# doesburg11/PredPreyGrass

Hardware: NVIDIA B200
Metric: agent_steps_per_s_incl_obs (higher is better)
Workload: dtype f64

## Files before the change

### predpreygrass_b200/csrc/ppg_api.cu

```cuda
#include <cuda_runtime.h>

#include <algorithm>
#include <cmath>
#include <cstdio>
#include <cstdlib>
#include <cstring>
#include <string>
#include <vector>

#include "ppg_device.cuh"

namespace ppg {
cudaError_t launch_step_base(const StepParams& p, int warps_per_cta, int n_cta, size_t smem, cudaStream_t stream);
cudaError_t step_base_occupancy(int warps_per_cta, int map_bytes, bool bulk, bool split, size_t smem, int* blocks_per_sm);
cudaError_t launch_prepare_offsets(const EnvHdr* hdr, int B, int n0, int n1, unsigned long long* cntA, unsigned long long* sum1,
                                   unsigned long long* sum2, int32_t* totals4, unsigned epoch, int hdr_founders, cudaStream_t s);
cudaError_t launch_init_hdr(EnvHdr* hdr, int B, unsigned long long seed, cudaStream_t s);
cudaError_t launch_relabel_rows(const StepParams& p, const unsigned long long* cntA, const unsigned long long* sum1,
                                const unsigned long long* sum2, const int32_t* totals4, cudaStream_t s);
cudaError_t launch_mark_reset(EnvHdr* hdr, int B, const unsigned long long* seeds, const uint8_t* mask, cudaStream_t s);
cudaError_t launch_set_tape(EnvHdr* hdr, int B, const long long* cell_off, cudaStream_t s);
cudaError_t launch_random_actions(const int32_t* n_rows, const int32_t* re0, const int32_t* ra0, const int32_t* re1,
                                  const int32_t* ra1, int32_t* a0, int32_t* a1, unsigned long long seed, unsigned call,
                                  unsigned n_actions, unsigned env_base, int blocks, cudaStream_t s);
// ... 6 lines not shown
cudaError_t launch_eco_founders(const StepParams& p, cudaStream_t s);
cudaError_t launch_step_stag(const StepParams& p, int n_cta, size_t smem, cudaStream_t stream);
cudaError_t step_stag_occupancy(int map_bytes, bool split, size_t smem, int* blocks_per_sm);
cudaError_t launch_set_tape_reals_stag(StagHdr* shdr, int B, const long long* real_off, cudaStream_t s);
cudaError_t launch_random_actions_stag(const int32_t* n_rows, const int32_t* re0, const int32_t* ra0, const int32_t* re1, const int32_t* ra1,
                                       int32_t* a0, int32_t* a1, unsigned long long seed, unsigned call, unsigned env_base, int t2_pred,
                                       int t2_prey, int ar0, int ar1, int blocks, cudaStream_t s);
}

namespace ppg { int g_pdl_chain = -1; }

using namespace ppg;

__global__ void ppg_pow_selftest_kernel(const double* __restrict__ x, const double* __restrict__ y, double* __restrict__ out, long long n) {
  for (long long i = (long long)blockIdx.x * blockDim.x + threadIdx.x; i < n; i += (long long)gridDim.x * blockDim.x) out[i] = ppg_pow(x[i], y[i]);
}

struct ppg_handle_s {
  ppg_config cfg;
  int B = 0, device = 0;
  StepParams P;
  std::vector<int32_t> walls;
  int warps_per_cta = 4, n_cta = 0;
  size_t smem_bytes = 0;
  unsigned long long launches_step = 0;
  unsigned long long ticket_next = 0;
  unsigned long long obs_ticket_next = 0;
  int n_cta_obs = 0;
  bool obs_overlap = true;
  unsigned long long q_next = 0;
  bool profiling = false;
  std::vector<cudaEvent_t> prof_events;
  unsigned long long calls = 0;
  int64_t launch_count = 0;
  std::vector<void*> allocs;
  unsigned long long* d_stats = nullptr;
  int32_t* d_tape_cells = nullptr;
  long long* d_tape_off = nullptr;
  double* d_tape_reals = nullptr;
  long long* d_tape_real_off = nullptr;
  uint8_t* d_mask = nullptr;
  unsigned long long* d_seeds = nullptr;
  int32_t* d_act[2] = {nullptr, nullptr};
  int32_t h_n_rows[4] = {0, 0, 0, 0};
  bool h_n_rows_valid = false;
  ppg_buffers bufs;
  size_t state_bytes = 0;
  std::string err;
};

static thread_local std::string g_err;

#define CK(call)                                                                             \
  do {                                                                                       \
    cudaError_t _e = (call);                                                                 \
    if (_e != cudaSuccess) {                                                                 \
      h->err = std::string(#call) + ": " + cudaGetErrorString(_e);                           \
      return PPG_ERR_CUDA;                                                                   \
    }                                                                                        \
  } while (0)

template <typename T>
static cudaError_t dalloc(ppg_handle h, T** p, size_t n) {
  void* q = nullptr;
  cudaError_t e = cudaMalloc(&q, std::max<size_t>(n, 1) * sizeof(T));
  if (e != cudaSuccess) return e;
// ... 409 lines not shown
    if (lpt) { for (int q = 0; q < 2; ++q) CKC(dalloc(h, &P.perm[q], (size_t)B)); CKC(dalloc(h, &P.perm_tag, 2)); CKC(dalloc(h, &P.perm_cursor, 4)); CKC(cudaMemset(P.perm_tag, 0xFF, 2 * sizeof(unsigned))); }
  }
  if (eco) {
    CKC(dalloc(h, &P.ehdr, (size_t)B));
    if (c.track_episode_sums) CKC(dalloc(h, &P.ep_sums, (size_t)B * PPG_EP_STRIDE));
    CKC(dalloc(h, &P.gh_n, (size_t)B)); CKC(dalloc(h, &P.gh_cell, (size_t)B * PPG_MAX_GHOSTS)); CKC(dalloc(h, &P.gh_val, (size_t)B * PPG_MAX_GHOSTS));
  }
  if (stag) CKC(dalloc(h, &P.shdr, (size_t)B));
  CKC(dalloc(h, &P.gr_pos, (size_t)B * std::max(1, P.n_grass)));
  CKC(dalloc(h, &P.gr_e, (size_t)B * std::max(1, P.n_grass)));
  CKC(dalloc(h, &P.counters, (size_t)B * PPG_N_STATS));
  CKC(dalloc(h, &P.ticket, 1));
  CKC(dalloc(h, &P.env_cycles, (size_t)B));
  if (P.obs_split) {
    void* q = nullptr;
    CKC(cudaMalloc(&q, (size_t)B * (size_t)P.img_stride));
    h->allocs.push_back(q);
    P.obs_img = static_cast<unsigned char*>(q);
    for (int s = 0; s < 2; ++s) CKC(dalloc(h, &P.nb_info[s], (size_t)B * P.cap[s]));
    CKC(dalloc(h, &P.obs_ticket, 1));
    CKC(dalloc(h, &P.queue, (size_t)B));
    CKC(dalloc(h, &P.q_tail, 1));
    if (const char* ev = getenv("PPG_OBS_OVERLAP")) h->obs_overlap = atoi(ev) != 0;
    if (eco)
      for (int s = 0; s < 2; ++s) CKC(dalloc(h, &P.born_obs[s], (size_t)B * PPG_BORN_K * (size_t)P.elems[s]));
    int per_sm = 0, n_sm = 0;
    CKC(obs_occupancy(P, &per_sm));
    CKC(cudaDeviceGetAttribute(&n_sm, cudaDevAttrMultiProcessorCount, device));
    if (per_sm < 1) { h->err = "observation kernel does not fit on an SM"; return fail(PPG_ERR_INVALID); }
    h->n_cta_obs = std::min(B, per_sm * n_sm);
    if (const char* ev = getenv("PPG_OBS_CTAS_PER_SM")) h->n_cta_obs = std::max(1, std::min(h->n_cta_obs, atoi(ev) * n_sm));
    if (const char* ev = getenv("PPG_STEP_CTAS_PER_SM")) h->n_cta = std::max(1, std::min(h->n_cta, atoi(ev) * n_sm));
  }
  CKC(dalloc(h, &P.error, 1));
  CKC(dalloc(h, &h->d_stats, PPG_N_STATS));
  CKC(dalloc(h, &h->d_mask, (size_t)B));
  CKC(dalloc(h, &h->d_seeds, (size_t)B));
  ppg_buffers& b = h->bufs;
  memset(&b, 0, sizeof b);
  for (int s = 0; s < 2; ++s) {
    const size_t rows = (size_t)B * P.cap[s];
    b.row_capacity[s] = (int64_t)rows;
    b.obs_row_elems[s] = P.elems[s];
    void* q = nullptr;
    CKC(cudaMalloc(&q, rows * (size_t)P.elems[s] * sizeof(float)));
    h->allocs.push_back(q);
    P.obs[s] = b.obs[s] = static_cast<float*>(q);
    CKC(dalloc(h, &P.row_env[s], rows)); CKC(dalloc(h, &P.row_agent[s], rows));
    CKC(dalloc(h, &P.reward[s], rows)); CKC(dalloc(h, &P.flags[s], rows));
    CKC(dalloc(h, &P.old_off[s], (size_t)B + 1)); CKC(dalloc(h, &P.new_off[s], (size_t)B + 1));
    CKC(dalloc(h, &P.new_cnt[s], (size_t)B + 1));
    CKC(dalloc(h, &h->d_act[s], rows));
    b.row_env[s] = P.row_env[s]; b.row_agent[s] = P.row_agent[s]; b.reward[s] = P.reward[s]; b.flags[s] = P.flags[s];
    b.old_off[s] = P.old_off[s]; b.new_off[s] = P.new_off[s]; b.new_cnt[s] = P.new_cnt[s];
  }
  CKC(dalloc(h, &P.n_rows, 4)); CKC(dalloc(h, &P.env_flags, (size_t)B)); CKC(dalloc(h, &P.env_status, (size_t)B));
  CKC(dalloc(h, &P.env_step, (size_t)B)); CKC(dalloc(h, &P.env_count, (size_t)B * 2));
  b.n_rows = P.n_rows; b.env_flags = P.env_flags; b.env_status = P.env_status; b.env_step = P.env_step; b.env_count = P.env_count;
  b.n_envs = B;
  CKC(launch_init_hdr(P.hdr, B, c.seed, 0));
  h->launch_count++;
  CKC(cudaDeviceSynchronize());
  *out = h;
  return PPG_OK;
#undef CKC
}
// ... 27 lines not shown
    h->P.tape_cells = h->d_tape_cells;
  }
  CK(launch_set_tape(h->P.hdr, h->B, h->d_tape_off, 0));
  h->launch_count++;
  if (h->P.variant == PPG_VARIANT_ECO || h->P.variant == PPG_VARIANT_STAG) {
    if (h->d_tape_reals) { cudaFree(h->d_tape_reals); h->d_tape_reals = nullptr; }
    if (h->d_tape_real_off) { cudaFree(h->d_tape_real_off); h->d_tape_real_off = nullptr; }
    h->P.tape_reals = nullptr;
    if (t && t->reals && t->real_off) {
      const int64_t total = t->real_off[h->B];
      CK(cudaMalloc(&h->d_tape_reals, sizeof(double) * (size_t)std::max<int64_t>(total, 1)));
      CK(cudaMalloc(&h->d_tape_real_off, sizeof(long long) * ((size_t)h->B + 1)));
      CK(cudaMemcpy(h->d_tape_reals, t->reals, sizeof(double) * (size_t)total, cudaMemcpyHostToDevice));
      CK(cudaMemcpy(h->d_tape_real_off, t->real_off, sizeof(long long) * ((size_t)h->B + 1), cudaMemcpyHostToDevice));
      h->P.tape_reals = h->d_tape_reals;
    }
    if (h->P.variant == PPG_VARIANT_ECO) CK(launch_set_tape_reals(h->P.ehdr, h->B, h->d_tape_real_off, 0));
    else CK(launch_set_tape_reals_stag(h->P.shdr, h->B, h->d_tape_real_off, 0));
    h->launch_count++;
  }
  CK(cudaDeviceSynchronize());
  return PPG_OK;
}

static int prepare_offsets(ppg_handle h, cudaStream_t st) {
  const unsigned prev_epoch = (unsigned)h->launches_step;
  const int q = (int)(prev_epoch & 1u);
  CK(launch_prepare_offsets(h->P.hdr, h->B, h->P.n_init[0], h->P.n_init[1], h->P.cntA[q], h->P.sum1[q], h->P.sum2[q],
                            h->P.totals + 4 * q, prev_epoch, h->P.variant == PPG_VARIANT_ECO && ppg_random_founders(h->P.trait_mode), st));
  h->launch_count++;
  return PPG_OK;
}

static int run_step_kernel(ppg_handle h, const int32_t* a0, const int32_t* a1, const int32_t* o0, const int32_t* o1, cudaStream_t st) {
  StepParams& P = h->P;
  P.actions[0] = a0; P.actions[1] = a1;
  P.order[0] = o0; P.order[1] = o1;
  P.ticket_base = h->ticket_next;
  P.static_first = (h->warps_per_cta == 1 && P.obs_split && P.variant != PPG_VARIANT_ECO) ? 1 : 0;
  if (const char* ev = getenv("PPG_STATIC_FIRST")) P.static_first = P.static_first && atoi(ev) != 0;
  h->ticket_next += P.static_first ? (unsigned long long)h->B
                    : h->warps_per_cta == 1 ? (unsigned long long)h->B + (unsigned long long)h->n_cta
                                          : (unsigned long long)((h->B + h->warps_per_cta - 1) / h->warps_per_cta) + (unsigned long long)h->n_cta;
  P.epoch = (unsigned)(h->launches_step + 1);
  P.q_base = h->q_next;
  if (P.obs_split) h->q_next += (unsigned long long)h->B;
  cudaEvent_t pe[3] = {nullptr, nullptr, nullptr};
  if (h->profiling) {
    for (int k = 0; k < 3; ++k) { CK(cudaEventCreate(&pe[k])); h->prof_events.push_back(pe[k]); }
    CK(cudaEventRecord(pe[0], st));
  }
  if (P.variant == PPG_VARIANT_ECO) CK(launch_step_eco(P, h->n_cta, h->smem_bytes, st));
  else if (P.variant == PPG_VARIANT_STAG) CK(launch_step_stag(P, h->n_cta, h->smem_bytes, st));
  else CK(launch_step_base(P, h->warps_per_cta, h->n_cta, h->smem_bytes, st));
  h->launches_step++;
  h->launch_count++;
  if (h->profiling) CK(cudaEventRecord(pe[1], st));
  if (P.obs_split) {
    P.obs_ticket_base = h->obs_ticket_next;
    h->obs_ticket_next += (unsigned long long)h->B + (unsigned long long)h->n_cta_obs;
    CK(launch_obs(P, h->n_cta_obs, h->obs_overlap && !h->profiling, st));
    h->launch_count++;
  }
  if (h->profiling) CK(cudaEventRecord(pe[2], st));
  h->calls++;
  h->h_n_rows_valid = false;
  return PPG_OK;
}

// ... 86 lines not shown

int ppg_random_actions(ppg_handle h, uint64_t seed, int32_t* actions_pred, int32_t* actions_prey, void* cuda_stream) {
  if (!h || !actions_pred || !actions_prey) return PPG_ERR_INVALID;
  CK(cudaSetDevice(h->device));
  const StepParams& P = h->P;
  if (P.variant == PPG_VARIANT_STAG)
    CK(launch_random_actions_stag(P.n_rows, P.row_env[0], P.row_agent[0], P.row_env[1], P.row_agent[1], actions_pred, actions_prey, seed,
                                  (unsigned)h->calls, (unsigned)P.env_base, P.n_possible_t[0][0], P.n_possible_t[1][0], P.type_ar[0], P.type_ar[1],
                                  148 * 4, static_cast<cudaStream_t>(cuda_stream)));
  else
  CK(launch_random_actions(P.n_rows, P.row_env[0], P.row_agent[0], P.row_env[1], P.row_agent[1], actions_pred, actions_prey,
                           seed, (unsigned)h->calls, (unsigned)P.n_actions, (unsigned)P.env_base, 148 * 4, static_cast<cudaStream_t>(cuda_stream)));
  h->launch_count++;
  return PPG_OK;
}

int ppg_set_pdl_chain(int32_t on) {
  const int before = pdl_chain_enabled() ? 1 : 0;
  g_pdl_chain = on ? 1 : 0;
  return before;
}

int ppg_rollout_random(ppg_handle* handles, int32_t n_handles, void** cuda_streams, int32_t n_steps, uint64_t seed) {
  if (!handles || n_handles <= 0 || n_steps < 0) return PPG_ERR_INVALID;
  struct ChainOff { int before; bool off; ChainOff(bool o) : before(pdl_chain_enabled()), off(o) { if (off) g_pdl_chain = 0; } ~ChainOff() { if (off) g_pdl_chain = before; } } chain_off(n_handles > 1);
  for (int g = 0; g < n_handles; ++g) {
    if (!handles[g]) return PPG_ERR_INVALID;
    if (handles[g]->launches_step == 0) { handles[g]->err = "ppg_rollout_random before ppg_reset"; return PPG_ERR_STATE; }
  }
  for (int k = 0; k < n_steps; ++k)
    for (int g = 0; g < n_handles; ++g) {
      ppg_handle h = handles[g];
      void* st = cuda_streams ? cuda_streams[g] : nullptr;
      int rc = ppg_random_actions(h, seed, h->d_act[0], h->d_act[1], st);
      if (rc) return rc;
      rc = run_step_kernel(h, h->d_act[0], h->d_act[1], nullptr, nullptr, static_cast<cudaStream_t>(st));
      if (rc) return rc;
    }
  return PPG_OK;
}

int ppg_selftest_pow(const double* x, const double* y, double* out, int64_t n, int32_t device) {
  if (!x || !y || !out || n <= 0) return PPG_ERR_INVALID;
  if (cudaSetDevice(device) != cudaSuccess) { g_err = "ppg_selftest_pow: bad device"; return PPG_ERR_NO_DEVICE; }
  double *dx = nullptr, *dy = nullptr, *dz = nullptr;
  const size_t bytes = (size_t)n * sizeof(double);
  cudaError_t e = cudaMalloc(&dx, bytes);
  if (e == cudaSuccess) e = cudaMalloc(&dy, bytes);
  if (e == cudaSuccess) e = cudaMalloc(&dz, bytes);
  if (e == cudaSuccess) e = cudaMemcpy(dx, x, bytes, cudaMemcpyHostToDevice);
  if (e == cudaSuccess) e = cudaMemcpy(dy, y, bytes, cudaMemcpyHostToDevice);
  if (e == cudaSuccess) { ppg_pow_selftest_kernel<<<148 * 8, 256>>>(dx, dy, dz, (long long)n); e = cudaGetLastError(); }
  if (e == cudaSuccess) e = cudaMemcpy(out, dz, bytes, cudaMemcpyDeviceToHost);
  cudaFree(dx); cudaFree(dy); cudaFree(dz);
  if (e != cudaSuccess) { g_err = std::string("ppg_selftest_pow: ") + cudaGetErrorString(e); return PPG_ERR_CUDA; }
  return PPG_OK;
}

int ppg_get_buffers(ppg_handle h, ppg_buffers* out) {
  if (!h || !out) return PPG_ERR_INVALID;
  *out = h->bufs;
  return PPG_OK;
}

struct Seg { void* p; size_t bytes; };
static std::vector<Seg> state_segments(ppg_handle h) {
// ... 323 lines not shown
```

### predpreygrass_b200/csrc/ppg_base.cu

```cuda
#include <cuda_runtime.h>

#include "ppg_step_common.cuh"

#ifndef PPG_MIN_CTAS
#define PPG_MIN_CTAS 20
#endif

namespace ppg {

PHASE_DEFINE(base)
SPAN_DEFINE(base)

#define SEL(a) (s == 0 ? a[0] : a[1])

template <int W, typename MapT, bool BULK, bool SPLIT>
__global__ void __launch_bounds__(W * 32, PPG_MIN_CTAS / W) ppg_step_base_kernel(const __grid_constant__ StepParams p) {
  extern __shared__ __align__(128) unsigned char smem_raw[];
  __shared__ int s_env0;
  const int warp = threadIdx.x >> 5, lane = threadIdx.x & 31;
  SPAN_MARK(base, 0)
  wait_for_stream_predecessor();
  if (SPLIT) allow_dependent_launch();
  unsigned char* const sbase = smem_raw + (size_t)warp * p.smem_per_env;
  const EnvSmem<MapT> S = carve<MapT>(sbase, p);
  const RowDesc D = carve_desc(sbase, p);
  const unsigned sb32 = (unsigned)__cvta_generic_to_shared(sbase);
  const int G = p.G, GG = p.GG, PP = p.P, PS = p.PS;
  const unsigned epoch = p.epoch;
  const int par = (int)(epoch & 1u);
  const int mode_r = p.reward_mode;
  const bool dense = mode_r == PPG_REWARD_DENSE || mode_r == PPG_REWARD_DENSE_ADDITIVE;
  const bool kick = mode_r == PPG_REWARD_SPARSE_KICKBACK;
  const unsigned lt_mask = (1u << lane) - 1u;

  {
    const int n16 = p.init_bytes / 16;
    #pragma unroll 1
    for (int i0 = 0; i0 < n16; i0 += 32 * 8) {
      uint4 v[8];
#pragma unroll
      for (int q = 0; q < 8; ++q) { const int i = i0 + 32 * q + lane; if (i < n16) v[q] = __ldg(reinterpret_cast<const uint4*>(p.init_image) + i); }
#pragma unroll
      for (int q = 0; q < 8; ++q) { const int i = i0 + 32 * q + lane; if (i < n16) reinterpret_cast<uint4*>(sbase + p.so_map[0])[i] = v[q]; }
    }
  }
  unsigned rowctr = 0;
  const int n_old_total[2] = {p.totals[(par ^ 1) * 4 + 0], p.totals[(par ^ 1) * 4 + 1]};
  const int n_blk = (p.B + 31) >> 5, n_grp = (p.B + 1023) >> 10;
// ... 108 lines not shown
            S.pos[s][i] = (uint16_t)((cx << 8) | cy);
            S.E[s][i] = p.init_e[s];
            S.flg[s][i] = F_ALIVE;
            if (kick) S.par[s][i] = 0xFFFF;
            S.ord[s][i] = (uint16_t)i;
            S.map[s][CELLXY(cx, cy)] = (MapT)(i + 1);
          }
          k0 += p.n_init[s];
          n[s] = p.n_init[s];
          h.n_list[s] = (unsigned short)p.n_init[s];
          h.n_sorted[s] = (unsigned short)p.n_init[s];
          h.next_idx[s] = (unsigned short)p.n_init[s];
        }
        #pragma unroll 1
        for (int g = lane; g < p.n_grass; g += 32) {
          const int c = cells[k0 + g];
          const int cx = c / G, cy = c % G;
          S.gpos[g] = (uint16_t)((cx << 8) | cy);
          S.gE[g] = p.grass_cap;
          S.map[2][CELLXY(cx, cy)] = (MapT)(g + 1);
        }
      }
      __syncwarp();
      cur[0] = n[0]; cur[1] = n[1];
      next_live[0] = n[0]; next_live[1] = n[1];
      env_flags = PPG_ENV_RESET;
      PHASE_MARK(2)
    } else if (mode == 2) {
      n[0] = h.n_list[0]; n[1] = h.n_list[1];
      int act_r[3] = {4, 4, 4};
#pragma unroll
      for (int q = 0; q < 3; ++q) {
        const int s = q ? 1 : 0, i = lane + (q == 2 ? 32 : 0);
        if (i < SEL(n)) act_r[q] = p.actions[s][prow_r[q]];
      }
      {
        const double grass_gain = p.season_len > 0 ? p.grass_gain_season[(h.step / p.season_len) & 1] : p.grass_gain;
#pragma unroll
        for (int q = 0; q < 4; ++q) {
          const int g = lane + 32 * q;
          if (g < p.n_grass) {
            S.gpos[g] = (uint16_t)gp_r[q];
            const double v = ge_r[q] + grass_gain;
            S.gE[g] = v < p.grass_cap ? v : p.grass_cap;
            S.map[2][CELLP(gp_r[q])] = (MapT)(g + 1);
          }
        }
        #pragma unroll 1
        for (int g = lane + 128; g < p.n_grass; g += 32) {
          const size_t b = (size_t)env * p.n_grass;
          const unsigned gp = p.gr_pos[b + g];
          S.gpos[g] = (uint16_t)gp;
          const double v = p.gr_e[b + g] + grass_gain;
          S.gE[g] = v < p.grass_cap ? v : p.grass_cap;
          S.map[2][CELLP(gp)] = (MapT)(g + 1);
        }
      }
      PHASE_MARK(4)
      unsigned bad = 0;
      bool resort[2] = {false, false};
#pragma unroll 1
      for (int s = 0; s < 2; ++s) {
        const size_t b = (size_t)env * p.cap[s];
        const int32_t* ordp = p.order[s];
        bool use_order = ordp != nullptr;
        if (PPG_UNLIKELY(use_order)) {
          bool ok = true;
          #pragma unroll 1
          for (int i = lane; i < SEL(n); i += 32) {
            const int d = ordp[p.ag_prow[s][b + i]];
            if ((unsigned)d < (unsigned)SEL(n)) SEL(S.rnk)[d] = (uint16_t)i; else ok = false;
          }
          __syncwarp();
          #pragma unroll 1
          for (int i = lane; i < SEL(n); i += 32) {
            const int d = ordp[p.ag_prow[s][b + i]];
            if ((unsigned)d < (unsigned)SEL(n)) ok &= SEL(S.rnk)[d] == (uint16_t)i;
          }
          use_order = __all_sync(FULL, ok);
          if (!use_order) bad = PPG_STATUS_BAD_ACTION;
          __syncwarp();
        }
        if (s == 0) resort[0] = use_order; else resort[1] = use_order;
        #pragma unroll 1
        for (int i = lane; i < SEL(n); i += 32) {
          const int q = s == 0 ? (i < 32 ? 0 : 3) : (i < 32 ? 1 : (i < 64 ? 2 : 3));
          int prow, a;
          double e;
          unsigned idpos, par16 = 0;
          if (q < 3) {
            prow = q == 0 ? prow_r[0] : (q == 1 ? prow_r[1] : prow_r[2]);
            e = q == 0 ? e_r[0] : (q == 1 ? e_r[1] : e_r[2]);
            idpos = q == 0 ? idpos_r[0] : (q == 1 ? idpos_r[1] : idpos_r[2]);
            a = q == 0 ? act_r[0] : (q == 1 ? act_r[1] : act_r[2]);
            if (kick) par16 = q == 0 ? par_r[0] : (q == 1 ? par_r[1] : par_r[2]);
          } else {
            prow = p.ag_prow[s][b + i];
            e = p.ag_e[s][b + i];
            idpos = (unsigned)p.ag_id[s][b + i] | ((unsigned)p.ag_pos[s][b + i] << 16);
            a = p.actions[s][prow];
            if (kick) par16 = p.ag_par[s][b + i];
          }
          const int d = use_order ? ordp[prow] : i;
          if ((unsigned)a > 8u) { a = 4; bad = PPG_STATUS_BAD_ACTION; }
          SEL(S.id)[d] = (uint16_t)idpos;
          SEL(S.pos)[d] = (uint16_t)(idpos >> 16);
          if (dense) SEL(S.E0)[d] = e;
          SEL(S.E)[d] = e - p.loss[s];
          SEL(S.act)[d] = (uint8_t)a;
          SEL(S.flg)[d] = F_ALIVE;
          SEL(S.ord)[d] = (uint16_t)d;
          SEL(S.rnk)[d] = (uint16_t)d;
          if (kick) { SEL(S.par)[d] = (uint16_t)par16; SEL(S.aux)[d] = 0; }
        }
      }
      h.status |= (unsigned char)__reduce_or_sync(FULL, bad);
      PHASE_MARK(3)
      __syncwarp();
#pragma unroll 1
      for (int s = 0; s < 2; ++s)
        for (int b0 = 0; b0 < SEL(n); b0 += 32) {
          const int i = b0 + lane;
          const bool v = i < SEL(n);
          int cell = 0;
          if (v) { cell = CELLP((unsigned)SEL(S.pos)[i]); SEL(S.map)[cell] = (MapT)(i + 1); }
          __syncwarp();
          bool need = v && SEL(S.map)[cell] < (unsigned)(i + 1);
          while (__any_sync(FULL, need)) {
            if (need) SEL(S.map)[cell] = (MapT)(i + 1);
            __syncwarp();
            need = v && SEL(S.map)[cell] < (unsigned)(i + 1);
          }
        }
// ... 600 lines not shown
  if (e >= B) return;
  EnvHdr h = {};
  h.seed_key = seed;
  h.state = ST_IDLE;
  hdr[e] = h;
}

__global__ void ppg_mark_reset_kernel(EnvHdr* hdr, int B, const unsigned long long* seeds, const uint8_t* mask) {
  const int e = blockIdx.x * blockDim.x + threadIdx.x;
  if (e >= B) return;
  if (mask && !mask[e]) return;
  if (seeds) hdr[e].seed_key = seeds[e];
  hdr[e].state = ST_NEEDS_RESET;
}

__global__ void ppg_set_tape_kernel(EnvHdr* hdr, int B, const long long* cell_off) {
  const int e = blockIdx.x * blockDim.x + threadIdx.x;
  if (e >= B) return;
  hdr[e].tape_pos = cell_off ? cell_off[e] : 0;
  hdr[e].tape_end = cell_off ? cell_off[e + 1] : 0;
}

__global__ void ppg_random_actions_kernel(const int32_t* __restrict__ n_rows, const int32_t* __restrict__ row_env0,
                                          const int32_t* __restrict__ row_agent0, const int32_t* __restrict__ row_env1,
                                          const int32_t* __restrict__ row_agent1, int32_t* act0, int32_t* act1,
                                          unsigned long long seed, unsigned call, unsigned n_actions, unsigned env_base) {
  allow_dependent_launch();
  wait_for_stream_predecessor();
  const volatile int32_t* const nr = n_rows;
  const int n0 = nr[0] + nr[2], n1 = nr[1] + nr[3];
  for (int i = blockIdx.x * blockDim.x + threadIdx.x; i < n0 + n1; i += gridDim.x * blockDim.x) {
    const int s = i >= n0;
    const int row = s ? i - n0 : i;
    const unsigned env = (unsigned)(s ? row_env1[row] : row_env0[row]) + env_base;
    const unsigned id = (unsigned)(s ? row_agent1[row] : row_agent0[row]);
    const unsigned r = ppg_draw_u32(seed, env, call, PPG_STREAM_ACTION + 8u * (unsigned)s, id);
    (s ? act1 : act0)[row] = (int32_t)ppg_bounded(r, n_actions);
  }
}

__global__ void ppg_stats_kernel(const uint32_t* __restrict__ counters, const EnvHdr* __restrict__ hdr, int B,
                                 unsigned long long* out) {
  __shared__ unsigned long long s_acc[PPG_N_STATS];
  if (threadIdx.x < PPG_N_STATS) s_acc[threadIdx.x] = 0;
  __syncthreads();
  const int k = threadIdx.x & (PPG_N_STATS - 1);
  unsigned long long a = 0;
  for (size_t i = (size_t)blockIdx.x * blockDim.x + threadIdx.x; i < (size_t)B * PPG_N_STATS; i += (size_t)gridDim.x * blockDim.x) {
    unsigned v = counters[i];
    if (k == PPG_STAT_STATUS_ENVS) v = hdr[i / PPG_N_STATS].status != 0;
    a += v;
  }
  atomicAdd(&s_acc[k], a);
  __syncthreads();
  if (threadIdx.x < PPG_N_STATS && s_acc[threadIdx.x]) atomicAdd(out + threadIdx.x, s_acc[threadIdx.x]);
}

template <int W, typename MapT, bool BULK, bool SPLIT>
static cudaError_t launch_w(const StepParams& p, int n_cta, size_t smem, cudaStream_t stream) {
  static size_t attr_bytes = 0;
  if (smem > attr_bytes) {
    cudaError_t e = cudaFuncSetAttribute(ppg_step_base_kernel<W, MapT, BULK, SPLIT>, cudaFuncAttributeMaxDynamicSharedMemorySize, (int)smem);
    if (e != cudaSuccess) return e;
    attr_bytes = smem;
  }
  return pdl_launch(ppg_step_base_kernel<W, MapT, BULK, SPLIT>, dim3((unsigned)n_cta), dim3(W * 32), smem, stream, p);
}

template <int W, typename MapT, bool BULK, bool SPLIT>
static cudaError_t occupancy_w(size_t smem, int* blocks_per_sm) {
  cudaError_t e = cudaFuncSetAttribute(ppg_step_base_kernel<W, MapT, BULK, SPLIT>, cudaFuncAttributeMaxDynamicSharedMemorySize, (int)smem);
  if (e != cudaSuccess) return e;
  return cudaOccupancyMaxActiveBlocksPerMultiprocessor(blocks_per_sm, ppg_step_base_kernel<W, MapT, BULK, SPLIT>, W * 32, smem);
}

#define PPG_DISPATCH(FN, ...)                                                                     \
  do {                                                                                            \
    const bool m8 = map_bytes == 1;                                                               \
    if (split) return m8 ? FN<1, uint8_t, false, true>(__VA_ARGS__) : FN<1, uint16_t, false, true>(__VA_ARGS__); \
    if (warps_per_cta == 1) {                                                                     \
      if (bulk) return m8 ? FN<1, uint8_t, true, false>(__VA_ARGS__) : FN<1, uint16_t, true, false>(__VA_ARGS__); \
      return m8 ? FN<1, uint8_t, false, false>(__VA_ARGS__) : FN<1, uint16_t, false, false>(__VA_ARGS__);       \
    }                                                                                             \
    if (warps_per_cta == 4) {                                                                     \
      if (bulk) return m8 ? FN<4, uint8_t, true, false>(__VA_ARGS__) : FN<4, uint16_t, true, false>(__VA_ARGS__); \
      return m8 ? FN<4, uint8_t, false, false>(__VA_ARGS__) : FN<4, uint16_t, false, false>(__VA_ARGS__);       \
    }                                                                                             \
    if (warps_per_cta == 8) {                                                                     \
      if (bulk) return m8 ? FN<8, uint8_t, true, false>(__VA_ARGS__) : FN<8, uint16_t, true, false>(__VA_ARGS__); \
      return m8 ? FN<8, uint8_t, false, false>(__VA_ARGS__) : FN<8, uint16_t, false, false>(__VA_ARGS__);       \
    }                                                                                             \
    return cudaErrorInvalidValue;                                                                 \
  } while (0)

cudaError_t launch_step_base(const StepParams& p, int warps_per_cta, int n_cta, size_t smem, cudaStream_t stream) {
  const int map_bytes = p.map_bytes;
  const bool bulk = p.obs_bulk != 0, split = p.obs_split != 0;
  PPG_DISPATCH(launch_w, p, n_cta, smem, stream);
}

cudaError_t step_base_occupancy(int warps_per_cta, int map_bytes, bool bulk, bool split, size_t smem, int* blocks_per_sm) {
  PPG_DISPATCH(occupancy_w, smem, blocks_per_sm);
}

cudaError_t launch_prepare_offsets(const EnvHdr* hdr, int B, int n0, int n1, unsigned long long* cntA, unsigned long long* sum1,
                                   unsigned long long* sum2, int32_t* totals4, unsigned epoch, int hdr_founders, cudaStream_t s) {
// ... 32 lines not shown
```

### predpreygrass_b200/csrc/ppg_device.cuh

```cuda
#pragma once
#include <cuda_runtime.h>
#include <stdint.h>

#include <cstdlib>
#include <utility>

#include "../../include/ppg.h"
#include "../../include/ppg_philox.h"
#include "../../include/ppg_pow.h"

namespace ppg {

#define PPG_MAX_NJ 13

struct __align__(16) EnvHdr {
  unsigned long long seed_key;
  long long tape_pos, tape_end;
  int step;
  unsigned episode;
  unsigned spawn_draws;
  unsigned short n_list[2];
  unsigned short next_idx[2];
  unsigned char state;
  unsigned char status;
// ... 59 lines not shown
  double loss[2], thr[2], init_e[2], grass_cap, grass_gain, init_e_grass;
  double grass_gain_season[2];
  int season_len;
  double r_catch, r_eat, r_pstep, r_qstep, pen_caught, r_repro[2], r_kick[2];
  EnvHdr* hdr;
  uint16_t* ag_id[2];
  uint16_t* ag_pos[2];
  double* ag_e[2];
  int32_t* ag_prow[2];
  uint16_t* ag_par[2];
  uint16_t* gr_pos;
  double* gr_e;
  const uint16_t* lexrank[2];
  const int32_t* tape_cells;
  uint32_t* counters;
  unsigned long long* ticket;
  unsigned long long ticket_base;
  int static_first;
  unsigned epoch;
  unsigned* error;
  unsigned long long* cntA[2];
  unsigned long long* cntB[2];
  unsigned long long* sum1[2];
  unsigned long long* sum2[2];
  unsigned long long* acc1;
  unsigned long long* acc2;
  unsigned long long* acc3;
  int32_t* totals;
  int32_t* perm[2];
  unsigned* perm_tag;
  unsigned* perm_cursor;
  const int32_t* order[2];
  const int32_t* actions[2];
  float* obs[2];
  int32_t* row_env[2];
  int32_t* row_agent[2];
  float* reward[2];
  uint8_t* flags[2];
  int32_t* old_off[2];
  int32_t* new_off[2];
  int32_t* new_cnt[2];
  int32_t* n_rows;
  uint8_t* env_flags;
  uint8_t* env_status;
  int32_t* env_step;
  int32_t* env_count;
  int so_E[2], so_E0[2], so_gE, so_wt, so_vt[3], so_stage, so_scr, so_id[2], so_pos[2], so_ord[2], so_rnk[2], so_par[2];
  int so_map[4], so_gpos, so_act[2], so_flg[2], so_aux[2], so_gtag;
  int stage_elems;
  int smem_per_env;
  int P, PS, CH;
  int map_bytes;
  int wall_idx;
  int nj[2];
  int obs_vec[2];
  int emit_kind[2];
  int obs_bulk;
  const void* init_image;
  int init_bytes;
  int variant, action_range, n_actions, genome_enabled, speed_in_obs, max_age[2], carcass_age, slow_dist, fast_dist;
  double move_cost[2], move_exp, bite_cap_grass, bite_cap_prey, f_mean[2], f_std[2], mut_rate, mut_std, sp_lo, sp_hi, sp_thr;
  EcoHdr* ehdr;
  uint16_t* ag_age[2];
  uint16_t* ag_seq[2];
  double* ag_spd[2];
  uint8_t* ag_dead[2];
// ... 66 lines not shown
```

### predpreygrass_b200/csrc/ppg_stag.cu

```cuda
#include <cuda_runtime.h>

#include "ppg_step_common.cuh"

namespace ppg {

#define SEL(a) (s == 0 ? a[0] : a[1])

static __device__ __noinline__ double capture_pow(double base, double exponent) { return ppg_pow(base, exponent); }

template <typename MapT>
struct StagSmem {
  MapT* map3;
  double* trait;
  uint8_t* face;
  uint8_t* join;
  uint16_t* age[2];
  uint16_t* mord[2];
  uint16_t* jl;
  uint16_t* rl;
};

template <typename MapT>
__device__ __forceinline__ StagSmem<MapT> carve_stag(unsigned char* base, const StepParams& p) {
  StagSmem<MapT> s;
// ... 988 lines not shown
    __syncwarp();
#if !PPG_PUSH_DEFER
    if (SPLIT) queue_push(p, pend, pend_env, lane);
#endif
#if !PPG_TICKET_EARLY
    if (lane == 0) {
      env_next = t_first + (int)(atomicAdd(p.ticket, 1ULL) - p.ticket_base);
      if (perm != nullptr && env_next < p.B) env_next = perm[env_next];
    }
#endif
  }
  if (SPLIT) queue_push(p, pend, pend_env, lane);
}

__global__ void ppg_set_tape_reals_stag_kernel(StagHdr* shdr, int B, const long long* real_off) {
  const int e = blockIdx.x * blockDim.x + threadIdx.x;
  if (e >= B) return;
  shdr[e].real_pos = real_off ? real_off[e] : 0;
  shdr[e].real_end = real_off ? real_off[e + 1] : 0;
}

__global__ void ppg_random_actions_stag_kernel(const int32_t* __restrict__ n_rows, const int32_t* __restrict__ row_env0,
                                               const int32_t* __restrict__ row_agent0, const int32_t* __restrict__ row_env1,
                                               const int32_t* __restrict__ row_agent1, int32_t* act0, int32_t* act1,
                                               unsigned long long seed, unsigned call, unsigned env_base, int t2_pred, int t2_prey,
                                               int ar0, int ar1) {
  allow_dependent_launch();
  wait_for_stream_predecessor();
  const volatile int32_t* const nr = n_rows;
  const int n0 = nr[0] + nr[2], n1 = nr[1] + nr[3];
  for (int i = blockIdx.x * blockDim.x + threadIdx.x; i < n0 + n1; i += gridDim.x * blockDim.x) {
    const int s = i >= n0;
    const int row = s ? i - n0 : i;
    const unsigned env = (unsigned)(s ? row_env1[row] : row_env0[row]) + env_base;
    const unsigned id = (unsigned)(s ? row_agent1[row] : row_agent0[row]);
    const unsigned r = ppg_draw_u32(seed, env, call, PPG_STREAM_ACTION + 8u * (unsigned)s, id);
    const int R = ((int)id >= (s ? t2_prey : t2_pred)) ? ar1 : ar0;
    const unsigned mv = ppg_bounded(r, (unsigned)(R > 0 ? R * R : 1));
    const unsigned jn = s == 0 ? (ppg_draw_u32(seed, env, call, PPG_STREAM_ACTION + 16u, id) & 1u) : 0u;
    (s ? act1 : act0)[row] = (int32_t)(mv | (jn << PPG_STAG_JOIN_SHIFT));
  }
}

template <typename MapT, bool SPLIT>
static cudaError_t launch_stag_t(const StepParams& p, int n_cta, size_t smem, cudaStream_t stream) {
  static size_t attr_bytes = 0;
  if (smem > attr_bytes) {
    cudaError_t e = cudaFuncSetAttribute(ppg_step_stag_kernel<1, MapT, SPLIT>, cudaFuncAttributeMaxDynamicSharedMemorySize, (int)smem);
    if (e != cudaSuccess) return e;
    attr_bytes = smem;
  }
  return pdl_launch(ppg_step_stag_kernel<1, MapT, SPLIT>, dim3((unsigned)n_cta), dim3(32), smem, stream, p);
}

cudaError_t launch_step_stag(const StepParams& p, int n_cta, size_t smem, cudaStream_t stream) {
  if (p.obs_split) return p.map_bytes == 1 ? launch_stag_t<uint8_t, true>(p, n_cta, smem, stream) : launch_stag_t<uint16_t, true>(p, n_cta, smem, stream);
  return p.map_bytes == 1 ? launch_stag_t<uint8_t, false>(p, n_cta, smem, stream) : launch_stag_t<uint16_t, false>(p, n_cta, smem, stream);
}

template <typename MapT, bool SPLIT>
static cudaError_t occupancy_stag_t(size_t smem, int* blocks_per_sm) {
  cudaError_t e = cudaFuncSetAttribute(ppg_step_stag_kernel<1, MapT, SPLIT>, cudaFuncAttributeMaxDynamicSharedMemorySize, (int)smem);
  if (e != cudaSuccess) return e;
  return cudaOccupancyMaxActiveBlocksPerMultiprocessor(blocks_per_sm, ppg_step_stag_kernel<1, MapT, SPLIT>, 32, smem);
}

cudaError_t step_stag_occupancy(int map_bytes, bool split, size_t smem, int* blocks_per_sm) {
  if (split) return map_bytes == 1 ? occupancy_stag_t<uint8_t, true>(smem, blocks_per_sm) : occupancy_stag_t<uint16_t, true>(smem, blocks_per_sm);
  return map_bytes == 1 ? occupancy_stag_t<uint8_t, false>(smem, blocks_per_sm) : occupancy_stag_t<uint16_t, false>(smem, blocks_per_sm);
}

cudaError_t launch_set_tape_reals_stag(StagHdr* shdr, int B, const long long* real_off, cudaStream_t s) {
  ppg_set_tape_reals_stag_kernel<<<(B + 255) / 256, 256, 0, s>>>(shdr, B, real_off);
// ... 12 lines not shown
```

### predpreygrass_b200/csrc/ppg_step_common.cuh

```cuda
#pragma once
#include <cuda_runtime.h>

#include "ppg_device.cuh"

namespace ppg {

#define FULL 0xffffffffu
#define PPG_UNLIKELY(x) __builtin_expect(!!(x), 0)

#ifndef PPG_TICKET_EARLY
#define PPG_TICKET_EARLY 1
#endif
#ifndef PPG_PUSH_DEFER
#define PPG_PUSH_DEFER 1
#endif

__device__ __forceinline__ void red_shared_add(const void* smem_ptr, unsigned v) {
  asm volatile("red.shared.add.u32 [%0], %1;" ::"r"((unsigned)__cvta_generic_to_shared(smem_ptr)), "r"(v) : "memory");
}
__device__ __forceinline__ int atom_shared_add(const void* smem_ptr, int v) {
  int old;
  asm volatile("atom.shared.add.s32 %0, [%1], %2;" : "=r"(old) : "r"((unsigned)__cvta_generic_to_shared(smem_ptr)), "r"(v) : "memory");
  return old;
}
// ... 112 lines not shown
  }
  return d;
}

__device__ __forceinline__ void dump_image(unsigned char* sbase, const StepParams& p, int env, int mode, bool keep, const int old_base[2],
                                           const int n[2], const int births[2], int lane) {
  int* ih = reinterpret_cast<int*>(sbase + p.so_ihdr);
  if (lane < IH_INTS) {
    int v = 0;
    switch (lane) {
      case IH_OLD_BASE0: v = old_base[0]; break;
      case IH_OLD_BASE1: v = old_base[1]; break;
      case IH_N0: v = mode ? n[0] : 0; break;
      case IH_N1: v = mode ? n[1] : 0; break;
      case IH_BIRTHS0: v = mode ? births[0] : 0; break;
      case IH_BIRTHS1: v = mode ? births[1] : 0; break;
      case IH_MODE: v = mode; break;
      case IH_KEEP: v = keep ? 1 : 0; break;
      default: break;
    }
    ih[lane] = v;
  }
  __syncwarp();
  const uint4* src = reinterpret_cast<const uint4*>(sbase + p.so_img);
  uint4* dst = reinterpret_cast<uint4*>(p.obs_img + (size_t)env * p.img_stride);
  const int n16 = mode ? p.img_bytes >> 4 : (IH_INTS * 4) >> 4;
  #pragma unroll 1
  for (int i = lane; i < n16; i += 32) dst[i] = src[i];
  __syncwarp();
}

__device__ __forceinline__ void allow_dependent_launch() { asm volatile("griddepcontrol.launch_dependents;" ::: "memory"); }
__device__ __forceinline__ void wait_for_stream_predecessor() { asm volatile("griddepcontrol.wait;" ::: "memory"); }


struct RowRel {
  int relb[PPG_MAX_NJ];
  unsigned tbl[PPG_MAX_NJ];
  unsigned self;
};

__device__ __forceinline__ RowRel load_rel(const StepParams& p, int s, unsigned sb32, int lane) {
  RowRel r;
  r.self = p.obs_self ? __ldg(p.obs_self + s * 32 + lane) : 0u;
#pragma unroll
  for (int j = 0; j < PPG_MAX_NJ; ++j) {
    r.relb[j] = 0; r.tbl[j] = 0;
    if (j < p.nj[s]) {
      const int2 v = __ldg(p.obs_rel + (s * PPG_MAX_NJ + j) * 32 + lane);
      r.relb[j] = v.x; r.tbl[j] = sb32 + (unsigned)v.y;
    }
  }
  return r;
}

template <typename MapT>
__device__ __forceinline__ void refresh_tables(const EnvSmem<MapT>& S, const StepParams& p, int nt0, int nt1, int lane) {
  #pragma unroll 1
  for (int i = lane; i < nt0; i += 32) S.vt[0][1 + i] = (float)S.E[0][i];
  #pragma unroll 1
  for (int i = lane; i < nt1; i += 32) S.vt[1][1 + i] = (float)S.E[1][i];
  #pragma unroll 1
  for (int g = lane; g < p.n_grass; g += 32) S.vt[2][1 + g] = (float)S.gE[g];
  if (lane == 0) S.vt[0][0] = 0.f;
  if (lane == 1) S.vt[1][0] = 0.f;
  if (lane == 2) S.vt[2][0] = 0.f;
// ... 483 lines not shown
```

Measured before the change: 1.549 billion.

## Fuse random action generation into base step kernel for random rollouts

In the random-rollout path, the step kernel for the base variant can now draw each agent's random action itself from (seed, call, env, species, id) instead of reading a buffer filled by a separate random-actions kernel. This removes one kernel launch per step and the global write and read of the action arrays. The draw logic is factored into a shared random_action helper that the standalone kernels also use, so both paths produce the same actions. It is only enabled for one warp per CTA, split-obs, non-bulk base configs with B at most twice the CTA count, and it adds a new template instantiation.

```diff
diff --git a/predpreygrass_b200/csrc/ppg_api.cu b/predpreygrass_b200/csrc/ppg_api.cu
--- a/predpreygrass_b200/csrc/ppg_api.cu
+++ b/predpreygrass_b200/csrc/ppg_api.cu
@@ -62,6 +62,7 @@
   bool profiling = false;
   std::vector<cudaEvent_t> prof_events;
   unsigned long long calls = 0;
+  bool draw_actions = false;
   int64_t launch_count = 0;
   std::vector<void*> allocs;
   unsigned long long* d_stats = nullptr;
@@ -537,6 +538,7 @@
     if (const char* ev = getenv("PPG_OBS_CTAS_PER_SM")) h->n_cta_obs = std::max(1, std::min(h->n_cta_obs, atoi(ev) * n_sm));
     if (const char* ev = getenv("PPG_STEP_CTAS_PER_SM")) h->n_cta = std::max(1, std::min(h->n_cta, atoi(ev) * n_sm));
   }
+  h->draw_actions = !eco && !stag && P.obs_split && !P.obs_bulk && W == 1 && (long long)B <= 2LL * h->n_cta;
   CKC(dalloc(h, &P.error, 1));
   CKC(dalloc(h, &h->d_stats, PPG_N_STATS));
   CKC(dalloc(h, &h->d_mask, (size_t)B));
@@ -630,9 +632,13 @@
   return PPG_OK;
 }
 
-static int run_step_kernel(ppg_handle h, const int32_t* a0, const int32_t* a1, const int32_t* o0, const int32_t* o1, cudaStream_t st) {
+static int run_step_kernel(ppg_handle h, const int32_t* a0, const int32_t* a1, const int32_t* o0, const int32_t* o1, cudaStream_t st,
+                           bool draw = false, unsigned long long act_seed = 0ULL) {
   StepParams& P = h->P;
   P.actions[0] = a0; P.actions[1] = a1;
+  P.act_draw = draw ? 1 : 0;
+  P.act_seed = act_seed;
+  P.act_call = (unsigned)h->calls;
   P.order[0] = o0; P.order[1] = o1;
   P.ticket_base = h->ticket_next;
   P.static_first = (h->warps_per_cta == 1 && P.obs_split && P.variant != PPG_VARIANT_ECO) ? 1 : 0;
@@ -785,6 +791,11 @@
     for (int g = 0; g < n_handles; ++g) {
       ppg_handle h = handles[g];
       void* st = cuda_streams ? cuda_streams[g] : nullptr;
+      if (h->draw_actions) {
+        const int rc = run_step_kernel(h, nullptr, nullptr, nullptr, nullptr, static_cast<cudaStream_t>(st), true, seed);
+        if (rc) return rc;
+        continue;
+      }
       int rc = ppg_random_actions(h, seed, h->d_act[0], h->d_act[1], st);
       if (rc) return rc;
       rc = run_step_kernel(h, h->d_act[0], h->d_act[1], nullptr, nullptr, static_cast<cudaStream_t>(st));
diff --git a/predpreygrass_b200/csrc/ppg_base.cu b/predpreygrass_b200/csrc/ppg_base.cu
--- a/predpreygrass_b200/csrc/ppg_base.cu
+++ b/predpreygrass_b200/csrc/ppg_base.cu
@@ -13,7 +13,7 @@
 
 #define SEL(a) (s == 0 ? a[0] : a[1])
 
-template <int W, typename MapT, bool BULK, bool SPLIT>
+template <int W, typename MapT, bool BULK, bool SPLIT, bool DRAW>
 __global__ void __launch_bounds__(W * 32, PPG_MIN_CTAS / W) ppg_step_base_kernel(const __grid_constant__ StepParams p) {
   extern __shared__ __align__(128) unsigned char smem_raw[];
   __shared__ int s_env0;
@@ -188,7 +188,9 @@
 #pragma unroll
       for (int q = 0; q < 3; ++q) {
         const int s = q ? 1 : 0, i = lane + (q == 2 ? 32 : 0);
-        if (i < SEL(n)) act_r[q] = p.actions[s][prow_r[q]];
+        if (i < SEL(n))
+          act_r[q] = DRAW ? random_action<false>(p.act_seed, p.act_call, (unsigned)p.env_base, env, s, idpos_r[q] & 0xFFFFu, (unsigned)p.n_actions, 0, 0, 0)
+                          : p.actions[s][prow_r[q]];
       }
       {
         const double grass_gain = p.season_len > 0 ? p.grass_gain_season[(h.step / p.season_len) & 1] : p.grass_gain;
@@ -254,7 +256,8 @@
             prow = p.ag_prow[s][b + i];
             e = p.ag_e[s][b + i];
             idpos = (unsigned)p.ag_id[s][b + i] | ((unsigned)p.ag_pos[s][b + i] << 16);
-            a = p.actions[s][prow];
+            a = DRAW ? random_action<false>(p.act_seed, p.act_call, (unsigned)p.env_base, env, s, idpos & 0xFFFFu, (unsigned)p.n_actions, 0, 0, 0)
+                     : p.actions[s][prow];
             if (kick) par16 = p.ag_par[s][b + i];
           }
           const int d = use_order ? ordp[prow] : i;
@@ -921,10 +924,9 @@
   for (int i = blockIdx.x * blockDim.x + threadIdx.x; i < n0 + n1; i += gridDim.x * blockDim.x) {
     const int s = i >= n0;
     const int row = s ? i - n0 : i;
-    const unsigned env = (unsigned)(s ? row_env1[row] : row_env0[row]) + env_base;
+    const int env = s ? row_env1[row] : row_env0[row];
     const unsigned id = (unsigned)(s ? row_agent1[row] : row_agent0[row]);
-    const unsigned r = ppg_draw_u32(seed, env, call, PPG_STREAM_ACTION + 8u * (unsigned)s, id);
-    (s ? act1 : act0)[row] = (int32_t)ppg_bounded(r, n_actions);
+    (s ? act1 : act0)[row] = random_action<false>(seed, call, env_base, env, s, id, n_actions, 0, 0, 0);
   }
 }
 
@@ -945,22 +947,31 @@
   if (threadIdx.x < PPG_N_STATS && s_acc[threadIdx.x]) atomicAdd(out + threadIdx.x, s_acc[threadIdx.x]);
 }
 
+template <int W, typename MapT, bool BULK, bool SPLIT, bool DRAW>
+static cudaError_t launch_k(const StepParams& p, int n_cta, size_t smem, cudaStream_t stream) {
+  static size_t attr_bytes = 0;
+  if (smem > attr_bytes) {
+    cudaError_t e = cudaFuncSetAttribute(ppg_step_base_kernel<W, MapT, BULK, SPLIT, DRAW>, cudaFuncAttributeMaxDynamicSharedMemorySize, (int)smem);
+    if (e != cudaSuccess) return e;
+    attr_bytes = smem;
+  }
+  return pdl_launch(ppg_step_base_kernel<W, MapT, BULK, SPLIT, DRAW>, dim3((unsigned)n_cta), dim3(W * 32), smem, stream, p);
+}
+
 template <int W, typename MapT, bool BULK, bool SPLIT>
 static cudaError_t launch_w(const StepParams& p, int n_cta, size_t smem, cudaStream_t stream) {
-  static size_t attr_bytes = 0;
-  if (smem > attr_bytes) {
-    cudaError_t e = cudaFuncSetAttribute(ppg_step_base_kernel<W, MapT, BULK, SPLIT>, cudaFuncAttributeMaxDynamicSharedMemorySize, (int)smem);
-    if (e != cudaSuccess) return e;
-    attr_bytes = smem;
-  }
-  return pdl_launch(ppg_step_base_kernel<W, MapT, BULK, SPLIT>, dim3((unsigned)n_cta), dim3(W * 32), smem, stream, p);
+  if constexpr (W == 1 && !BULK && SPLIT) {
+    if (p.act_draw) return launch_k<W, MapT, BULK, SPLIT, true>(p, n_cta, smem, stream);
+  }
+  if (p.act_draw) return cudaErrorInvalidValue;
+  return launch_k<W, MapT, BULK, SPLIT, false>(p, n_cta, smem, stream);
 }
 
 template <int W, typename MapT, bool BULK, bool SPLIT>
 static cudaError_t occupancy_w(size_t smem, int* blocks_per_sm) {
-  cudaError_t e = cudaFuncSetAttribute(ppg_step_base_kernel<W, MapT, BULK, SPLIT>, cudaFuncAttributeMaxDynamicSharedMemorySize, (int)smem);
+  cudaError_t e = cudaFuncSetAttribute(ppg_step_base_kernel<W, MapT, BULK, SPLIT, false>, cudaFuncAttributeMaxDynamicSharedMemorySize, (int)smem);
   if (e != cudaSuccess) return e;
-  return cudaOccupancyMaxActiveBlocksPerMultiprocessor(blocks_per_sm, ppg_step_base_kernel<W, MapT, BULK, SPLIT>, W * 32, smem);
+  return cudaOccupancyMaxActiveBlocksPerMultiprocessor(blocks_per_sm, ppg_step_base_kernel<W, MapT, BULK, SPLIT, false>, W * 32, smem);
 }
 
 #define PPG_DISPATCH(FN, ...)                                                                     \
diff --git a/predpreygrass_b200/csrc/ppg_device.cuh b/predpreygrass_b200/csrc/ppg_device.cuh
--- a/predpreygrass_b200/csrc/ppg_device.cuh
+++ b/predpreygrass_b200/csrc/ppg_device.cuh
@@ -115,6 +115,9 @@
   unsigned* perm_cursor;
   const int32_t* order[2];
   const int32_t* actions[2];
+  int act_draw;
+  unsigned act_call;
+  unsigned long long act_seed;
   float* obs[2];
   int32_t* row_env[2];
   int32_t* row_agent[2];
diff --git a/predpreygrass_b200/csrc/ppg_stag.cu b/predpreygrass_b200/csrc/ppg_stag.cu
--- a/predpreygrass_b200/csrc/ppg_stag.cu
+++ b/predpreygrass_b200/csrc/ppg_stag.cu
@@ -1044,13 +1044,9 @@
   for (int i = blockIdx.x * blockDim.x + threadIdx.x; i < n0 + n1; i += gridDim.x * blockDim.x) {
     const int s = i >= n0;
     const int row = s ? i - n0 : i;
-    const unsigned env = (unsigned)(s ? row_env1[row] : row_env0[row]) + env_base;
+    const int env = s ? row_env1[row] : row_env0[row];
     const unsigned id = (unsigned)(s ? row_agent1[row] : row_agent0[row]);
-    const unsigned r = ppg_draw_u32(seed, env, call, PPG_STREAM_ACTION + 8u * (unsigned)s, id);
-    const int R = ((int)id >= (s ? t2_prey : t2_pred)) ? ar1 : ar0;
-    const unsigned mv = ppg_bounded(r, (unsigned)(R > 0 ? R * R : 1));
-    const unsigned jn = s == 0 ? (ppg_draw_u32(seed, env, call, PPG_STREAM_ACTION + 16u, id) & 1u) : 0u;
-    (s ? act1 : act0)[row] = (int32_t)(mv | (jn << PPG_STAG_JOIN_SHIFT));
+    (s ? act1 : act0)[row] = random_action<true>(seed, call, env_base, env, s, id, 0u, s ? t2_prey : t2_pred, ar0, ar1);
   }
 }
 
diff --git a/predpreygrass_b200/csrc/ppg_step_common.cuh b/predpreygrass_b200/csrc/ppg_step_common.cuh
--- a/predpreygrass_b200/csrc/ppg_step_common.cuh
+++ b/predpreygrass_b200/csrc/ppg_step_common.cuh
@@ -168,6 +168,18 @@
 
 __device__ __forceinline__ void allow_dependent_launch() { asm volatile("griddepcontrol.launch_dependents;" ::: "memory"); }
 __device__ __forceinline__ void wait_for_stream_predecessor() { asm volatile("griddepcontrol.wait;" ::: "memory"); }
+
+template <bool STAG>
+__device__ __forceinline__ int random_action(unsigned long long seed, unsigned call, unsigned env_base, int env, int s, unsigned id,
+                                             unsigned n_actions, int t2, int ar0, int ar1) {
+  const unsigned genv = (unsigned)env + env_base;
+  const unsigned r = ppg_draw_u32(seed, genv, call, PPG_STREAM_ACTION + 8u * (unsigned)s, id);
+  if (!STAG) return (int)ppg_bounded(r, n_actions);
+  const int R = (int)id >= t2 ? ar1 : ar0;
+  const unsigned mv = ppg_bounded(r, (unsigned)(R > 0 ? R * R : 1));
+  const unsigned jn = s == 0 ? (ppg_draw_u32(seed, genv, call, PPG_STREAM_ACTION + 16u, id) & 1u) : 0u;
+  return (int)(mv | (jn << PPG_STAG_JOIN_SHIFT));
+}
 
 
 struct RowRel {
```

Result: faster. 1.658 billion (median of 6 runs) (+7.0%).
